# Windere/EAS-SNN

Hardware: AMD Instinct MI355X
Metric: event-frames/sec (T=3) SYOLOX-S Gen1 304x240 (higher is better)
Workload: dtype f32

## Files before the change

eas_snn_amd/csrc/bn_act.hip:

```cpp
#include "eas_common.h"

namespace {

constexpr int NW = EAS_BLOCK / EAS_WAVE;

__device__ __forceinline__ float silu(float z) { return z * eas_sigmoidf(z); }
__device__ __forceinline__ float silu_grad(float z) {
    const float sg = eas_sigmoidf(z);
    return sg * (1.0f + z * (1.0f - sg));
}

__device__ __forceinline__ void bn_silu_fwd_body(const float* __restrict__ y, const float* __restrict__ mean,
                                                 const float* __restrict__ invstd, const float* __restrict__ gamma,
                                                 const float* __restrict__ beta, float* __restrict__ out, int N, int C, int HW, const BnFin& fin,
                                                 int out_ctot, int y_ctot, const int c, const int chunk, const int nchunks_g) {
    __shared__ float st[2];
    if (c >= C) return;
    const int hw4 = HW / EAS_VEC;
    const int64_t groups = (int64_t)N * hw4;
    float mu, istd;
    if (fin.part) {
        bn_finalize_in_block(fin, c, st, mu, istd, chunk == 0);
    } else {
        mu = mean[c];
        istd = invstd[c];
    }
    const float scale = gamma[c] * istd;
    const float shift = beta[c] - mu * scale;
    GroupWalk gw((int64_t)chunk * blockDim.x + threadIdx.x, (int64_t)nchunks_g * blockDim.x, hw4);
    for (int64_t g = (int64_t)chunk * blockDim.x + threadIdx.x; g < groups; g += (int64_t)nchunks_g * blockDim.x, gw.next()) {
        const int64_t n = gw.n;
        const int q = gw.q;
        const int64_t base = (n * C + c) * (int64_t)HW + (int64_t)q * EAS_VEC;
        const float4 v = *reinterpret_cast<const float4*>(y + (y_ctot ? (n * y_ctot + c) * (int64_t)HW + (int64_t)q * EAS_VEC : base));
        float4 o;
        o.x = silu(fmaf(v.x, scale, shift)); o.y = silu(fmaf(v.y, scale, shift));
        o.z = silu(fmaf(v.z, scale, shift)); o.w = silu(fmaf(v.w, scale, shift));
        *reinterpret_cast<float4*>(out + (out_ctot ? (n * out_ctot + c) * (int64_t)HW + (int64_t)q * EAS_VEC : base)) = o;
    }
}

__global__ __launch_bounds__(EAS_BLOCK) void bn_silu_fwd_kernel(const float* __restrict__ y, const float* __restrict__ mean,
                                                                const float* __restrict__ invstd,
                                                                const float* __restrict__ gamma,
                                                                const float* __restrict__ beta, float* __restrict__ out, int N,
                                                                int C, int HW, BnFin fin, int out_ctot, int y_ctot) {
    bn_silu_fwd_body(y, mean, invstd, gamma, beta, out, N, C, HW, fin, out_ctot, y_ctot, (int)(blockIdx.z * 8 + blockIdx.x), (int)blockIdx.y,
                     (int)gridDim.y);
}

template <bool APPLY>
__device__ __forceinline__ void bn_silu_bwd_body(const float* __restrict__ grad_out, const float* __restrict__ y,
                                                 const float* __restrict__ mean, const float* __restrict__ invstd,
                                                 const float* __restrict__ gamma, const float* __restrict__ beta,
                                                 int batch_stats, double* __restrict__ part, int nchunks,
                                                 float* __restrict__ grad_y, float* __restrict__ grad_gamma,
                                                 float* __restrict__ grad_beta, int N, int C, int HW, int go_ctot, int y_ctot, const int c,
                                                 const int chunk, const int nchunks_g) {
    __shared__ double red[NW];
    __shared__ float bc[2];
    if (c >= C) return;
    const float mu = mean[c], istd = invstd[c];
    const float scale = gamma[c] * istd;
    const float shift = beta[c] - mu * scale;
    const int hw4 = HW / EAS_VEC;
    const int64_t groups = (int64_t)N * hw4;
    float m1 = 0.f, m2 = 0.f;
    if (APPLY) bn_bwd_means<2>(part, c, nchunks, (double)N * HW, chunk, batch_stats, grad_beta, grad_gamma, bc, m1, m2);
    float s1 = 0.f, s2 = 0.f;
    GroupWalk gw((int64_t)chunk * blockDim.x + threadIdx.x, (int64_t)nchunks_g * blockDim.x, hw4);
    for (int64_t g = (int64_t)chunk * blockDim.x + threadIdx.x; g < groups; g += (int64_t)nchunks_g * blockDim.x, gw.next()) {
        const int64_t n = gw.n;
        const int q = gw.q;
        const int64_t base = (n * C + c) * (int64_t)HW + (int64_t)q * EAS_VEC;
        const int64_t ybase = y_ctot ? (n * y_ctot + c) * (int64_t)HW + (int64_t)q * EAS_VEC : base;
        const float4 yv = *reinterpret_cast<const float4*>(y + ybase);
        const float4 gv = *reinterpret_cast<const float4*>(grad_out + (go_ctot ? (n * go_ctot + c) * (int64_t)HW + (int64_t)q * EAS_VEC : base));
        const float ys[4] = {yv.x, yv.y, yv.z, yv.w};
        const float gs[4] = {gv.x, gv.y, gv.z, gv.w};
        float o[4];
#pragma unroll
        for (int e = 0; e < 4; ++e) {
            const float dz = gs[e] * silu_grad(fmaf(ys[e], scale, shift));
            const float xhat = bn_xhat(ys[e], mu, istd);
            if (APPLY) {
                o[e] = bn_bwd_apply(scale, dz, xhat, m1, m2);
            } else {
                s1 += dz;
                s2 += dz * xhat;
            }
        }
        if (APPLY) *reinterpret_cast<float4*>(grad_y + ybase) = make_float4(o[0], o[1], o[2], o[3]);
    }
    if (!APPLY) {
        const double t1 = eas_block_sum<double, NW>((double)s1, red);
        const double t2 = eas_block_sum<double, NW>((double)s2, red);
        if (threadIdx.x == 0) {
            part[((int64_t)c * EAS_BN_MAX_CHUNKS + chunk) * 2 + 0] = t1;
            part[((int64_t)c * EAS_BN_MAX_CHUNKS + chunk) * 2 + 1] = t2;
        }
    }
}

template <bool APPLY>
__global__ __launch_bounds__(EAS_BLOCK) void bn_silu_bwd_kernel(const float* __restrict__ grad_out, const float* __restrict__ y,
                                                                const float* __restrict__ mean, const float* __restrict__ invstd,
                                                                const float* __restrict__ gamma, const float* __restrict__ beta,
                                                                int batch_stats, double* __restrict__ part, int nchunks,
                                                                float* __restrict__ grad_y, float* __restrict__ grad_gamma,
                                                                float* __restrict__ grad_beta, int N, int C, int HW, int go_ctot, int y_ctot) {
    bn_silu_bwd_body<APPLY>(grad_out, y, mean, invstd, gamma, beta, batch_stats, part, nchunks, grad_y, grad_gamma, grad_beta, N, C, HW, go_ctot,
                            y_ctot, (int)(blockIdx.z * 8 + blockIdx.x), (int)blockIdx.y, (int)gridDim.y);
}

constexpr int kMaxBnGroup = 12;
struct BnSiluFwdGroup {
    const float* y[kMaxBnGroup];
    const float* mean[kMaxBnGroup];
    const float* invstd[kMaxBnGroup];
    const float* gamma[kMaxBnGroup];
    const float* beta[kMaxBnGroup];
    float* out[kMaxBnGroup];
    BnFin fin[kMaxBnGroup];
    int N[kMaxBnGroup], C[kMaxBnGroup], HW[kMaxBnGroup], out_ctot[kMaxBnGroup], y_ctot[kMaxBnGroup], chunks[kMaxBnGroup];
    int first[kMaxBnGroup + 1];
    int n;
};

template <class G>
__device__ __forceinline__ void bn_group_block(const G& a, int& p, int& c, int& chunk) {
    p = 0;
    for (int i = 1; i < a.n; ++i)
        if ((int)blockIdx.x >= a.first[i]) p = i;
    p = __builtin_amdgcn_readfirstlane(p);
    const int lb = (int)blockIdx.x - a.first[p];
    const int r = lb >> 3;
    chunk = r % a.chunks[p];
    c = (r / a.chunks[p]) * 8 + (lb & 7);
}

__global__ __launch_bounds__(EAS_BLOCK) void bn_silu_fwd_group_kernel(const BnSiluFwdGroup a) {
    int p, c, chunk;
    bn_group_block(a, p, c, chunk);
    bn_silu_fwd_body(a.y[p], a.mean[p], a.invstd[p], a.gamma[p], a.beta[p], a.out[p], a.N[p], a.C[p], a.HW[p], a.fin[p], a.out_ctot[p],
                     a.y_ctot[p], c, chunk, a.chunks[p]);
}

struct BnSiluBwdGroup {
    const float* grad_out[kMaxBnGroup];
    const float* y[kMaxBnGroup];
    const float* mean[kMaxBnGroup];
    const float* invstd[kMaxBnGroup];
// ... 92 lines not shown
    if (q.HW % EAS_VEC != 0 || q.C > 65535) return EAS_ERR_UNSUPPORTED;
    if (((uintptr_t)q.y | (uintptr_t)q.grad_out | (uintptr_t)q.grad_y) & 15) return EAS_ERR_INVALID_ARG;
    return EAS_OK;
}

static inline int bn_chan_blocks(int chunks, int C) { return 8 * chunks * ((C + 7) / 8); }

}

extern "C" {

int eas_bn_silu_fwd_ex(const float* y, float* mean, float* invstd, const float* gamma, const float* beta,
                       float* out, int N, int C, int HW, const EasBnPending* pend, int out_ctot, int y_ctot, eas_stream_t stream) {
    EasBnSiluFwdProblem q{y, mean, invstd, gamma, beta, out, N, C, HW, out_ctot, y_ctot, pend ? *pend : EasBnPending{}};
    BnFin fin;
    if (int rc = bn_silu_fwd_check(q, fin)) return rc;
    EAS_CLEAR_ERR();
    const int chunks = bn_pick_chunks((int64_t)N * (HW / EAS_VEC), C);
    EAS_LAUNCH(bn_silu_fwd_kernel, EAS_CHAN_GRID(chunks, C), dim3(EAS_BLOCK), 0, eas_s(stream), y, mean, invstd, gamma, beta, out, N, C, HW, fin,
               q.out_ctot, q.y_ctot);
    EAS_CHECK_LAUNCH();
    return EAS_OK;
}

int eas_bn_silu_fwd(const float* y, const float* mean, const float* invstd, const float* gamma, const float* beta,
                    float* out, int N, int C, int HW, eas_stream_t stream) {
    return eas_bn_silu_fwd_ex(y, const_cast<float*>(mean), const_cast<float*>(invstd), gamma, beta, out, N, C, HW, nullptr, 0, 0, stream);
}

int eas_bn_silu_bwd(const float* grad_out, const float* y, const float* mean, const float* invstd, const float* gamma,
                    const float* beta, int batch_stats, float* grad_y, float* grad_gamma, float* grad_beta,
                    double* workspace, int N, int C, int HW, int go_ctot, int y_ctot, eas_stream_t stream) {
    EasBnSiluBwdProblem q{grad_out, y, mean, invstd, gamma, beta, grad_y, grad_gamma, grad_beta, workspace, batch_stats, N, C, HW, go_ctot, y_ctot};
    if (int rc = bn_silu_bwd_check(q)) return rc;
    go_ctot = q.grad_out_ctot;
    y_ctot = q.y_ctot;
    hipStream_t st = eas_s(stream);
    EAS_CLEAR_ERR();
    {
        static const bool small_ok = !(eas_dev_env("EAS_BNSILU_BWD") && eas_dev_env("EAS_BNSILU_BWD")[0] == 't');
        constexpr int GPT = 6;
        const int64_t groups = (int64_t)N * (HW / EAS_VEC);
        if (small_ok && C >= 64 && groups <= 1024 * GPT) {
#define EAS_SMALL(NT_) EAS_LAUNCH((bn_silu_bwd_small_kernel<NT_, GPT>), dim3(C), dim3(NT_), 0, st, grad_out, y, mean, invstd, gamma, beta, \
                                           batch_stats, grad_y, grad_gamma, grad_beta, N, C, HW, go_ctot, y_ctot)
            if (groups <= 256 * GPT) EAS_SMALL(256);
            else if (groups <= 512 * GPT) EAS_SMALL(512);
            else EAS_SMALL(1024);
#undef EAS_SMALL
            EAS_CHECK_LAUNCH();
            return EAS_OK;
        }
    }
    const int chunks = bn_pick_chunks((int64_t)N * (HW / EAS_VEC), C);
    EAS_LAUNCH(bn_silu_bwd_kernel<false>, EAS_CHAN_GRID(chunks, C), dim3(EAS_BLOCK), 0, st, grad_out, y, mean, invstd, gamma, beta,
                       batch_stats, workspace, chunks, grad_y, grad_gamma, grad_beta, N, C, HW, go_ctot, y_ctot);
    EAS_CHECK_LAUNCH();
    EAS_LAUNCH(bn_silu_bwd_kernel<true>, EAS_CHAN_GRID(chunks, C), dim3(EAS_BLOCK), 0, st, grad_out, y, mean, invstd, gamma, beta,
                       batch_stats, workspace, chunks, grad_y, grad_gamma, grad_beta, N, C, HW, go_ctot, y_ctot);
    EAS_CHECK_LAUNCH();
    return EAS_OK;
}

int eas_bn_silu_fwd_group(const EasBnSiluFwdProblem* pr, int n, eas_stream_t stream) {
    if (!pr || n < 1) return EAS_ERR_INVALID_ARG;
    if (n > kMaxBnGroup) return EAS_ERR_UNSUPPORTED;
    BnSiluFwdGroup a{};
    int blocks = 0;
    for (int p = 0; p < n; ++p) {
        EasBnSiluFwdProblem q = pr[p];
        if (int rc = bn_silu_fwd_check(q, a.fin[p])) return rc;
        a.y[p] = q.y; a.mean[p] = q.mean; a.invstd[p] = q.invstd; a.gamma[p] = q.gamma; a.beta[p] = q.beta; a.out[p] = q.out;
        a.N[p] = q.N; a.C[p] = q.C; a.HW[p] = q.HW; a.out_ctot[p] = q.out_ctot; a.y_ctot[p] = q.y_ctot;
        a.chunks[p] = bn_pick_chunks((int64_t)q.N * (q.HW / EAS_VEC), q.C);
        a.first[p] = blocks;
        blocks += bn_chan_blocks(a.chunks[p], q.C);
    }
    a.first[n] = blocks;
    a.n = n;
    EAS_CLEAR_ERR();
    EAS_LAUNCH(bn_silu_fwd_group_kernel, dim3(blocks), dim3(EAS_BLOCK), 0, eas_s(stream), a);
    EAS_CHECK_LAUNCH();
    return EAS_OK;
}

int eas_bn_silu_bwd_group(const EasBnSiluBwdProblem* pr, int n, eas_stream_t stream) {
    if (!pr || n < 1) return EAS_ERR_INVALID_ARG;
    if (n > kMaxBnGroup) return EAS_ERR_UNSUPPORTED;
    BnSiluBwdGroup a{};
    int blocks = 0;
    for (int p = 0; p < n; ++p) {
        EasBnSiluBwdProblem q = pr[p];
        if (int rc = bn_silu_bwd_check(q)) return rc;
        a.grad_out[p] = q.grad_out; a.y[p] = q.y; a.mean[p] = q.mean; a.invstd[p] = q.invstd; a.gamma[p] = q.gamma; a.beta[p] = q.beta;
        a.part[p] = q.workspace; a.grad_y[p] = q.grad_y; a.grad_gamma[p] = q.grad_gamma; a.grad_beta[p] = q.grad_beta;
        a.batch_stats[p] = q.batch_stats; a.N[p] = q.N; a.C[p] = q.C; a.HW[p] = q.HW; a.go_ctot[p] = q.grad_out_ctot; a.y_ctot[p] = q.y_ctot;
        a.chunks[p] = bn_pick_chunks((int64_t)q.N * (q.HW / EAS_VEC), q.C);
        a.first[p] = blocks;
        blocks += bn_chan_blocks(a.chunks[p], q.C);
    }
    a.first[n] = blocks;
    a.n = n;
    EAS_CLEAR_ERR();
    EAS_LAUNCH(bn_silu_bwd_group_kernel<false>, dim3(blocks), dim3(EAS_BLOCK), 0, eas_s(stream), a);
    EAS_CHECK_LAUNCH();
    EAS_LAUNCH(bn_silu_bwd_group_kernel<true>, dim3(blocks), dim3(EAS_BLOCK), 0, eas_s(stream), a);
    EAS_CHECK_LAUNCH();
    return EAS_OK;
}

}
```

eas_snn_amd/csrc/bn_lif.hip:

```cpp
#include <stdlib.h>
#include <string.h>

#include "bn_lif_policy.h"
#include "eas_common.h"

namespace {

constexpr int NW = EAS_BLOCK / EAS_WAVE;

__global__ __launch_bounds__(EAS_BLOCK) void bn_stats_partial(const float* __restrict__ y, int TN, int C, int HW,
                                                              double* __restrict__ part, int Cy) {
    __shared__ double red[NW];
    const int c = blockIdx.y;
    const int hw4 = HW / EAS_VEC;
    const int64_t groups = (int64_t)TN * hw4;
    double s = 0.0, ss = 0.0;
    const int64_t stride = (int64_t)gridDim.x * blockDim.x;
    GroupWalk gw((int64_t)blockIdx.x * blockDim.x + threadIdx.x, stride, hw4);
    int64_t g = (int64_t)blockIdx.x * blockDim.x + threadIdx.x;
    for (; g + stride < groups; g += 2 * stride) {
        const float4 v0 = reinterpret_cast<const float4*>(y + (((int64_t)gw.n * Cy + c) * (int64_t)HW))[gw.q];
        gw.next();
        const float4 v1 = reinterpret_cast<const float4*>(y + (((int64_t)gw.n * Cy + c) * (int64_t)HW))[gw.q];
        gw.next();
// ... 185 lines not shown
                    acc[j][e] += s;
                    if (res_planes) s += (float)rp[e][j];
                    o[j] = (__bf16)s;
                }
                planes[(((int64_t)t * N + n) * out_groups_tot + grp) * (int64_t)HW + (int64_t)q * PV + e] = o;
            }
        }
#pragma unroll
        for (int j = 0; j < 8; ++j) {
            const int64_t base = (n * C + 8 * grp + j) * (int64_t)HW + (int64_t)q * PV;
            if (v_out) {
                vecp o;
#pragma unroll
                for (int e = 0; e < PV; ++e) o[e] = v[j][e];
                *reinterpret_cast<vecp*>(v_out + base) = o;
            }
            if (mean_out) {
                vecp o;
#pragma unroll
                for (int e = 0; e < PV; ++e) o[e] = acc[j][e] / Tf;
                *reinterpret_cast<vecp*>(mean_out + base) = o;
            }
        }
    }
}

template <int T_, bool HARD, bool DI, bool STRICT, class POL>
__device__ __forceinline__ void recompute_dz(const float (&yv)[T_], const float (&gs)[T_], float v0, float scale,
                                             float shift, float k, float omk, const EasLifParams& p, bool detach,
                                             int sg_id, float alpha, float (&dz)[T_], float& dk, float& da) {
    float h[T_], vprev[T_], z[T_];
    float v = v0;
#pragma unroll
    for (int t = 0; t < T_; ++t) {
        float s;
        vprev[t] = v;
        z[t] = fmaf(yv[t], scale, shift);
        eas_lif_step<HARD, DI, STRICT>(v, z[t], k, omk, p.v_th, p.v_reset, h[t], s);
    }
    float gv = 0.f;
#pragma unroll
    for (int t = T_ - 1; t >= 0; --t) {
        float dkt, gx;
        if constexpr (POL::fast)
            eas_lif_step_bwd_ct<HARD, DI, STRICT, POL::sg, POL::detach>(gs[t], gv, h[t], vprev[t], z[t], k, omk, p.v_th, p.v_reset, alpha, dkt,
                                                                        gx, da);
        else
            eas_lif_step_bwd<HARD, DI, STRICT>(gs[t], gv, h[t], vprev[t], z[t], k, omk, p.v_th, p.v_reset, detach, sg_id, alpha, dkt, gx, da);
        dz[t] = gx;
        dk += dkt;
    }
}

template <int T_, bool HARD, bool DI, bool STRICT, bool APPLY, class POL>
__global__ __launch_bounds__(EAS_BLOCK) void bn_lif_bwd_kernel(
    const float* __restrict__ grad_s, const float* __restrict__ grad_mean, const float* __restrict__ y,
    const float* __restrict__ mean, const float* __restrict__ invstd, const float* __restrict__ gamma,
    const float* __restrict__ beta, const float* __restrict__ v_init, EasLifParams p, int sg_id, float alpha,
    int batch_stats, double* __restrict__ part, int nchunks, float* __restrict__ grad_y, float* __restrict__ grad_gamma,
    float* __restrict__ grad_beta, float* __restrict__ grad_w, int N, int C, int HW, int bcast, int gs_ctot, int y_ctot,
    const float* __restrict__ alpha_dev, float* __restrict__ grad_alpha, int c_begin, int c_end, int finalize) {
    __shared__ double red[NW];
    __shared__ float bc[2];
    constexpr bool FAST = POL::fast;
    if (FAST) { bcast = 0; sg_id = POL::sg; }
    if (alpha_dev) alpha = fabsf(*alpha_dev);
    const int c = c_begin + blockIdx.z * 8 + blockIdx.x;
    if (c >= c_end) return;
    const int chunk = blockIdx.y, nchunks_g = gridDim.y;
    const float mu = mean[c], istd = invstd[c];
    const float scale = gamma[c] * istd;
    const float shift = beta[c] - mu * scale;
    const float k = eas_lif_k(p);
    const float omk = 1.0f - k;
    const bool detach = (p.flags & EAS_LIF_DETACH_RESET) != 0;
    const int hw4 = HW / EAS_VEC;
    const int64_t groups = (int64_t)N * hw4;
    const int64_t M = (int64_t)N * C * HW;
    const float invT = 1.0f / (float)T_;
    const int Cy = y_ctot ? y_ctot : C;
    const int64_t My = (int64_t)N * Cy * HW;
    const int64_t yts = bcast ? 0 : My;
    const int64_t Mg = gs_ctot ? (int64_t)N * gs_ctot * HW : M;
    const int Cg = gs_ctot ? gs_ctot : C;
    float m1 = 0.f, m2 = 0.f;
    if (APPLY) bn_bwd_means<4>(part, c, nchunks, (double)T_ * N * HW, chunk, batch_stats, grad_beta, grad_gamma, bc, m1, m2);
    float s1 = 0.f, s2 = 0.f, dk = 0.f, da = 0.f;
    GroupWalk gw((int64_t)chunk * blockDim.x + threadIdx.x, (int64_t)nchunks_g * blockDim.x, hw4);
    for (int64_t g = (int64_t)chunk * blockDim.x + threadIdx.x; g < groups; g += (int64_t)nchunks_g * blockDim.x, gw.next()) {
        const int64_t n = gw.n;
        const int q = gw.q;
        const int64_t base = (n * C + c) * (int64_t)HW + (int64_t)q * EAS_VEC;
        float4 ys[T_], gsv[T_];
        const int64_t ybase = (n * Cy + c) * (int64_t)HW + (int64_t)q * EAS_VEC;
#pragma unroll
        for (int t = 0; t < T_; ++t) ys[t] = *reinterpret_cast<const float4*>(y + (int64_t)t * yts + ybase);
        float4 gm = make_float4(0.f, 0.f, 0.f, 0.f);
        if (!FAST && grad_mean) {
            gm = *reinterpret_cast<const float4*>(grad_mean + base);
            gm.x *= invT; gm.y *= invT; gm.z *= invT; gm.w *= invT;
        }
#pragma unroll
        for (int t = 0; t < T_; ++t) {
            gsv[t] = gm;
            if (FAST || grad_s) {
                const int64_t gbase = FAST ? (n * Cg + c) * (int64_t)HW + (int64_t)q * EAS_VEC
                                           : (gs_ctot ? (n * gs_ctot + c) * (int64_t)HW + (int64_t)q * EAS_VEC : base);
                const float4 g4 = *reinterpret_cast<const float4*>(grad_s + (int64_t)t * Mg + gbase);
                gsv[t].x += g4.x; gsv[t].y += g4.y; gsv[t].z += g4.z; gsv[t].w += g4.w;
            }
        }
        const float vr0 = HARD ? p.v_reset : 0.0f;
        float4 v0 = make_float4(vr0, vr0, vr0, vr0);
        if (!FAST && v_init) v0 = *reinterpret_cast<const float4*>(v_init + base);
        float4 outv[T_];
#pragma unroll
        for (int e = 0; e < EAS_VEC; ++e) {
            float yv[T_], gs[T_], dz[T_];
#pragma unroll
            for (int t = 0; t < T_; ++t) {
                yv[t] = reinterpret_cast<const float*>(&ys[t])[e];
                gs[t] = reinterpret_cast<const float*>(&gsv[t])[e];
            }
            const float v0e = reinterpret_cast<const float*>(&v0)[e];
            float dke = 0.f;
            recompute_dz<T_, HARD, DI, STRICT, POL>(yv, gs, v0e, scale, shift, k, omk, p, detach, sg_id, alpha, dz, dke, da);
#pragma unroll
            for (int t = 0; t < T_; ++t) {
                const float xhat = bn_xhat(yv[t], mu, istd);
                if (APPLY) {
                    reinterpret_cast<float*>(&outv[t])[e] = bn_bwd_apply(scale, dz[t], xhat, m1, m2);
                } else {
                    s1 += dz[t];
                    s2 += dz[t] * xhat;
                }
            }
            dk += dke;
        }
        if (APPLY) {
            if (bcast) {
                float4 a = outv[0];
#pragma unroll
                for (int t = 1; t < T_; ++t) { a.x += outv[t].x; a.y += outv[t].y; a.z += outv[t].z; a.w += outv[t].w; }
                *reinterpret_cast<float4*>(grad_y + ybase) = a;
            } else {
#pragma unroll
                for (int t = 0; t < T_; ++t) *reinterpret_cast<float4*>(grad_y + (int64_t)t * My + ybase) = outv[t];
            }
        }
    }
    if (APPLY && finalize && chunk == 0 && c == c_begin) {
        auto slot = [&](int i, int k_) {
            const int cc = i / nchunks, j = i - cc * nchunks;
            return part[((int64_t)cc * EAS_BN_MAX_CHUNKS + j) * 4 + k_];
        };
        eas_lif_scalar_grads(C * nchunks, [&](int i) { return slot(i, 2); }, [&](int i) { return slot(i, 3); }, p.w_logit, alpha_dev, grad_w,
                             grad_alpha, red);
    }
    if (!APPLY) {
        const double t1 = eas_block_sum<double, NW>((double)s1, red);
        const double t2 = eas_block_sum<double, NW>((double)s2, red);
        const double t3 = eas_block_sum<double, NW>((double)dk, red);
        double t4 = 0.0;
        if (sg_id == EAS_SG_PATAN) t4 = eas_block_sum<double, NW>((double)da, red);
        if (threadIdx.x == 0) {
            double* o = part + ((int64_t)c * EAS_BN_MAX_CHUNKS + chunk) * 4;
            o[0] = t1; o[1] = t2; o[2] = t3; o[3] = t4;
        }
    }
}

template <int T_, bool HARD, bool DI, bool STRICT, int NT_, int GPT, class POL>
__global__ __launch_bounds__(NT_) void bn_lif_bwd_small_kernel(
    const float* __restrict__ grad_s, const float* __restrict__ grad_mean, const float* __restrict__ y,
    const float* __restrict__ mean, const float* __restrict__ invstd, const float* __restrict__ gamma,
    const float* __restrict__ beta, const float* __restrict__ v_init, EasLifParams p, int sg_id, float alpha,
    int batch_stats, double* __restrict__ part, float* __restrict__ grad_y, float* __restrict__ grad_gamma,
    float* __restrict__ grad_beta, int N, int C, int HW, int gs_ctot, int y_ctot, const float* __restrict__ alpha_dev) {
    constexpr int NWV = NT_ / EAS_WAVE;
    __shared__ double red[4][NWV];
    __shared__ float bc[2];
    if (POL::fast) sg_id = POL::sg;
    if (alpha_dev) alpha = fabsf(*alpha_dev);
    const int c = blockIdx.x;
    const float mu = mean[c], istd = invstd[c];
    const float scale = gamma[c] * istd;
    const float shift = beta[c] - mu * scale;
    const float k = eas_lif_k(p);
    const float omk = 1.0f - k;
    const bool detach = (p.flags & EAS_LIF_DETACH_RESET) != 0;
    const int hw4 = HW / EAS_VEC;
    const int groups = N * hw4;
    const int64_t M = (int64_t)N * C * HW;
    const int Cy = y_ctot ? y_ctot : C;
    const int64_t My = (int64_t)N * Cy * HW;
    const int64_t Mg = gs_ctot ? (int64_t)N * gs_ctot * HW : M;
    const float invT = 1.0f / (float)T_;
    float4 ys[GPT][T_], gsv[GPT][T_], v0[GPT];
    int64_t ybase[GPT];
#pragma unroll
    for (int i = 0; i < GPT; ++i) {
        const int g = threadIdx.x + i * NT_;
        const int gg = g < groups ? g : groups - 1;
        const int n = gg / hw4, q = gg - n * hw4;
        const int64_t base = ((int64_t)n * C + c) * (int64_t)HW + (int64_t)q * EAS_VEC;
        ybase[i] = ((int64_t)n * Cy + c) * (int64_t)HW + (int64_t)q * EAS_VEC;
#pragma unroll
        for (int t = 0; t < T_; ++t) ys[i][t] = *reinterpret_cast<const float4*>(y + (int64_t)t * My + ybase[i]);
        float4 gm = make_float4(0.f, 0.f, 0.f, 0.f);
        if (grad_mean) {
            gm = *reinterpret_cast<const float4*>(grad_mean + base);
            gm.x *= invT; gm.y *= invT; gm.z *= invT; gm.w *= invT;
        }
#pragma unroll
        for (int t = 0; t < T_; ++t) {
            gsv[i][t] = gm;
            if (grad_s) {
                const int64_t gbase = gs_ctot ? ((int64_t)n * gs_ctot + c) * (int64_t)HW + (int64_t)q * EAS_VEC : base;
                const float4 g4 = *reinterpret_cast<const float4*>(grad_s + (int64_t)t * Mg + gbase);
                gsv[i][t].x += g4.x; gsv[i][t].y += g4.y; gsv[i][t].z += g4.z; gsv[i][t].w += g4.w;
            }
        }
        const float vr0 = HARD ? p.v_reset : 0.0f;
        v0[i] = make_float4(vr0, vr0, vr0, vr0);
        if (v_init) v0[i] = *reinterpret_cast<const float4*>(v_init + base);
    }
    float sum[4] = {0.f, 0.f, 0.f, 0.f};
#pragma unroll
    for (int i = 0; i < GPT; ++i) {
        const bool live = threadIdx.x + i * NT_ < groups;
#pragma unroll
        for (int e = 0; e < EAS_VEC; ++e) {
            float yv[T_], gs[T_], dz[T_];
#pragma unroll
            for (int t = 0; t < T_; ++t) {
                yv[t] = reinterpret_cast<const float*>(&ys[i][t])[e];
                gs[t] = reinterpret_cast<const float*>(&gsv[i][t])[e];
            }
            float dke = 0.f, dae = 0.f;
            recompute_dz<T_, HARD, DI, STRICT, POL>(yv, gs, reinterpret_cast<const float*>(&v0[i])[e], scale, shift, k, omk, p, detach, sg_id, alpha, dz, dke, dae);
            if (live) {
#pragma unroll
                for (int t = 0; t < T_; ++t) {
                    sum[0] += dz[t];
                    sum[1] += dz[t] * bn_xhat(yv[t], mu, istd);
                }
                sum[2] += dke;
                sum[3] += dae;
            }
        }
    }
    double t[4];
    eas_block_totals<NWV, 4>(sum, red, t);
    if (threadIdx.x == 0) {
        bn_bwd_publish(t[0], t[1], (double)T_ * N * HW, true, c, grad_beta, grad_gamma, bc);
        double* o = part + ((int64_t)c * EAS_BN_MAX_CHUNKS) * 4;
        o[0] = t[0]; o[1] = t[1]; o[2] = t[2]; o[3] = sg_id == EAS_SG_PATAN ? t[3] : 0.0;
    }
    __syncthreads();
    const float m1 = batch_stats ? bc[0] : 0.f, m2 = batch_stats ? bc[1] : 0.f;
#pragma unroll
    for (int i = 0; i < GPT; ++i) {
        if (threadIdx.x + i * NT_ >= groups) continue;
        float4 outv[T_];
#pragma unroll
        for (int e = 0; e < EAS_VEC; ++e) {
            float yv[T_], gs[T_], dz[T_];
#pragma unroll
            for (int t = 0; t < T_; ++t) {
                yv[t] = reinterpret_cast<const float*>(&ys[i][t])[e];
                gs[t] = reinterpret_cast<const float*>(&gsv[i][t])[e];
            }
            float dke = 0.f, dae = 0.f;
            recompute_dz<T_, HARD, DI, STRICT, POL>(yv, gs, reinterpret_cast<const float*>(&v0[i])[e], scale, shift, k, omk, p, detach, sg_id, alpha, dz, dke, dae);
#pragma unroll
            for (int t = 0; t < T_; ++t) reinterpret_cast<float*>(&outv[t])[e] = bn_bwd_apply(scale, dz[t], bn_xhat(yv[t], mu, istd), m1, m2);
        }
#pragma unroll
        for (int t = 0; t < T_; ++t) *reinterpret_cast<float4*>(grad_y + (int64_t)t * My + ybase[i]) = outv[t];
    }
}

__global__ __launch_bounds__(EAS_BLOCK) void bn_lif_bwd_scalars_kernel(const double* __restrict__ part, int C, EasLifParams p, float* __restrict__ grad_w,
                                                                       const float* __restrict__ alpha_dev, float* __restrict__ grad_alpha) {
    __shared__ double red[NW];
    auto slot = [&](int i, int k_) { return part[((int64_t)i * EAS_BN_MAX_CHUNKS) * 4 + k_]; };
    eas_lif_scalar_grads(C, [&](int i) { return slot(i, 2); }, [&](int i) { return slot(i, 3); }, p.w_logit, alpha_dev, grad_w, grad_alpha, red);
}

template <int T_, bool HARD, bool DI, bool STRICT>
int launch_fwd_t(const float* y, const float* mean, const float* invstd, const float* gamma, const float* beta,
                 const float* v_in, float* v_out, EasLifParams p, float* spikes, float* mean_out, int N, int C, int HW,
                 int bcast, const BnFin& fin, const BnLifOut& ox, bf16x8* planes, const bf16x8* res_planes, int out_groups, int res_groups,
                 hipStream_t st) {
    if (planes) {
        if (fin.part) {
            EAS_LAUNCH(bn_finalize_kernel, dim3(C), dim3(EAS_BLOCK), 0, st, fin);
            EAS_CHECK_LAUNCH();
        }
        constexpr int PV = 1;
        const int chunks = bn_pick_chunks((int64_t)N * (HW / PV), C / 8);
        EAS_LAUNCH((bn_lif_fwd_sp_kernel<T_, HARD, DI, STRICT, PV>), EAS_CHAN_GRID(chunks, C / 8), dim3(EAS_BLOCK), 0, st, y,
                           mean, invstd, gamma, beta, v_in,
                           v_out, p, planes, res_planes, mean_out, N, C, HW, bcast, ox.y_ctot, out_groups, res_groups);
        EAS_CHECK_LAUNCH();
        return EAS_OK;
    }
    const int chunks = bn_pick_chunks((int64_t)N * (HW / EAS_VEC), C);
    EAS_LAUNCH((bn_lif_fwd_kernel<T_, HARD, DI, STRICT>), EAS_CHAN_GRID(chunks, C), dim3(EAS_BLOCK), 0, st, y, mean,
                       invstd, gamma, beta, v_in, v_out, p, spikes, mean_out, N, C, HW, bcast, fin, ox);
    EAS_CHECK_LAUNCH();
    return EAS_OK;
}

template <bool HARD, bool DI, bool STRICT>
int launch_fwd(int T, const float* y, const float* mean, const float* invstd, const float* gamma, const float* beta,
               const float* v_in, float* v_out, EasLifParams p, float* spikes, float* mean_out, int N, int C, int HW,
               int bcast, const BnFin& fin, const BnLifOut& ox, bf16x8* planes, const bf16x8* res_planes, int out_groups, int res_groups,
               hipStream_t st) {
#define EAS_CASE(TT) \
    case TT: return launch_fwd_t<TT, HARD, DI, STRICT>(y, mean, invstd, gamma, beta, v_in, v_out, p, spikes, mean_out, N, C, HW, bcast, fin, ox, planes, res_planes, out_groups, res_groups, st);
    switch (T) {
        EAS_CASE(1) EAS_CASE(2) EAS_CASE(3) EAS_CASE(4) EAS_CASE(5) EAS_CASE(6) EAS_CASE(7) EAS_CASE(8)
        default: return EAS_ERR_UNSUPPORTED;
    }
#undef EAS_CASE
}

struct BwdCall {
    const float *grad_s, *grad_mean, *y, *mean, *invstd, *gamma, *beta, *v_init;
    EasLifParams p;
    int sg;
    float alpha;
    int batch_stats;
    float *grad_y, *grad_gamma, *grad_beta, *grad_w;
    double* ws;
    int T, N, C, HW, bcast, gs_ctot, y_ctot;
    const float* alpha_dev;
    float* grad_alpha;
    hipStream_t st;
};

static inline bool bwd_form(const char* word) {
    const char* form = getenv("EAS_BNLIF_BWD");
    return form && strstr(form, word);
}

static inline int bwd_one_pass_gpt(const BwdCall& c) {
    const int gpt = c.T <= 3 ? 3 : (c.T <= 5 ? 2 : 1);
    const int64_t groups = (int64_t)c.N * (c.HW / EAS_VEC);
    return (!bwd_form("two") && !c.bcast && c.C >= 64 && groups <= 512 * gpt) ? gpt : 0;
}

template <int T_, bool HARD, bool DI, bool STRICT, class POL>
int launch_bwd_t(const BwdCall& c) {
    const int N = c.N, C = c.C, HW = c.HW;
    const int chunks = bn_pick_chunks((int64_t)N * (HW / EAS_VEC), C);
    if (bwd_one_pass_gpt(c)) {
        constexpr int GPT = T_ <= 3 ? 3 : (T_ <= 5 ? 2 : 1);
        const int64_t groups = (int64_t)N * (HW / EAS_VEC);
#define EAS_SMALL(NT_) EAS_LAUNCH((bn_lif_bwd_small_kernel<T_, HARD, DI, STRICT, NT_, GPT, POL>), dim3(C), dim3(NT_), 0, c.st, c.grad_s, c.grad_mean, c.y, \
                                   c.mean, c.invstd, c.gamma, c.beta, c.v_init, c.p, c.sg, c.alpha, c.batch_stats, c.ws, c.grad_y, c.grad_gamma,       \
                                   c.grad_beta, N, C, HW, c.gs_ctot, c.y_ctot, c.alpha_dev)
        if (groups <= 256 * GPT) EAS_SMALL(256);
        else EAS_SMALL(512);
#undef EAS_SMALL
        EAS_CHECK_LAUNCH();
        if (c.grad_w || c.grad_alpha) {
            EAS_LAUNCH(bn_lif_bwd_scalars_kernel, dim3(1), dim3(EAS_BLOCK), 0, c.st, c.ws, C, c.p, c.grad_w, c.alpha_dev, c.grad_alpha);
            EAS_CHECK_LAUNCH();
        }
        return EAS_OK;
    }
    static const int group_mb = eas_dev_env("EAS_BNLIF_BWD_GROUP_MB") ? atoi(eas_dev_env("EAS_BNLIF_BWD_GROUP_MB")) : 0;
    int gc = C;
    if (group_mb > 0) {
        const double per_channel = (double)N * HW * 4.0 * ((c.bcast ? 1 : T_) + T_);
        gc = (int)(group_mb * 1048576.0 / per_channel) / 8 * 8;
        if (gc < 8) gc = 8;
        if (gc > C) gc = C;
    }
    for (int c0 = 0; c0 < C; c0 += gc) {
        const int c1 = c0 + gc < C ? c0 + gc : C;
        const int last = c1 == C;
        EAS_LAUNCH((bn_lif_bwd_kernel<T_, HARD, DI, STRICT, false, POL>), EAS_CHAN_GRID(chunks, c1 - c0), dim3(EAS_BLOCK), 0, c.st, c.grad_s,
                   c.grad_mean, c.y, c.mean, c.invstd, c.gamma, c.beta, c.v_init, c.p, c.sg, c.alpha, c.batch_stats, c.ws, chunks, c.grad_y,
                   c.grad_gamma, c.grad_beta, (float*)nullptr, N, C, HW, c.bcast, c.gs_ctot, c.y_ctot, c.alpha_dev, (float*)nullptr, c0, c1, 0);
        EAS_CHECK_LAUNCH();
        EAS_LAUNCH((bn_lif_bwd_kernel<T_, HARD, DI, STRICT, true, POL>), EAS_CHAN_GRID(chunks, c1 - c0), dim3(EAS_BLOCK), 0, c.st, c.grad_s,
                   c.grad_mean, c.y, c.mean, c.invstd, c.gamma, c.beta, c.v_init, c.p, c.sg, c.alpha, c.batch_stats, c.ws, chunks, c.grad_y,
                   c.grad_gamma, c.grad_beta, c.grad_w, N, C, HW, c.bcast, c.gs_ctot, c.y_ctot, c.alpha_dev, c.grad_alpha, c0, c1, last);
        EAS_CHECK_LAUNCH();
    }
    return EAS_OK;
}

struct BwdRow {
    int T;
    bool hard, di;
    int sg;
    bool detach;
    int (*fn)(const BwdCall&);
};
template <int T_, bool HARD, bool DI, int SG = EAS_SG_RUNTIME, bool DETACH = false>
constexpr BwdRow bwd_row() {
    return {T_, HARD, DI, SG, DETACH, launch_bwd_t<T_, HARD, DI, false, BnLifBwdPolicy<SG, DETACH>>};
}
#define EAS_BWD_GENERIC_ROWS(H, D) \
    bwd_row<1, H, D>(), bwd_row<2, H, D>(), bwd_row<3, H, D>(), bwd_row<4, H, D>(), bwd_row<5, H, D>(), bwd_row<6, H, D>(), bwd_row<7, H, D>(), bwd_row<8, H, D>()
const BwdRow kBwdInstances[] = {
    bwd_row<3, false, false, EAS_SG_ATAN>(), bwd_row<5, false, false, EAS_SG_ATAN>(), bwd_row<7, false, false, EAS_SG_ATAN>(),
    EAS_BWD_GENERIC_ROWS(false, false), EAS_BWD_GENERIC_ROWS(true, false), EAS_BWD_GENERIC_ROWS(false, true), EAS_BWD_GENERIC_ROWS(true, true),
};
#undef EAS_BWD_GENERIC_ROWS

int bwd_select(const BwdCall& c) {
    const bool hard = c.p.flags & EAS_LIF_HARD_RESET, di = c.p.flags & EAS_LIF_DECAY_INPUT, detach = c.p.flags & EAS_LIF_DETACH_RESET;
    if (c.p.flags & EAS_LIF_FIRE_STRICT) return EAS_ERR_UNSUPPORTED;
    const bool plain = bwd_one_pass_gpt(c) || (c.grad_s && !c.grad_mean && !c.v_init && !c.bcast);
    const bool fast_ok = plain && !bwd_form("generic");
    for (const BwdRow& r : kBwdInstances) {
        if (r.T != c.T || r.hard != hard || r.di != di) continue;
        if (r.sg == EAS_SG_RUNTIME || (fast_ok && r.sg == c.sg && r.detach == detach)) return r.fn(c);
    }
    return EAS_ERR_UNSUPPORTED;
}
// ... 143 lines not shown
```

eas_snn_amd/csrc/eas_common.h:

```cpp
#pragma once
#include <hip/hip_runtime.h>
#include <stdint.h>
#include <stdlib.h>

#include <type_traits>

#include "../../include/eas_hip.h"

#define EAS_WAVE 64
#define EAS_BLOCK 256

#define EAS_CLEAR_ERR() (void)hipGetLastError()
#define EAS_CHECK_LAUNCH()                                          \
    do {                                                            \
        if (hipGetLastError() != hipSuccess) return EAS_ERR_LAUNCH; \
    } while (0)

static inline hipStream_t eas_s(eas_stream_t s) { return reinterpret_cast<hipStream_t>(s); }

__attribute__((visibility("hidden"))) extern int eas_trace_on;
__attribute__((visibility("hidden"))) extern long long eas_launch_count;
__attribute__((visibility("hidden"))) void eas_trace_kernel(const void* host_function);
#define EAS_LAUNCH(kern, ...)                                                \
    do {                                                                     \
// ... 118 lines not shown
                    s[p] += a;
                    q[p] = __builtin_elementwise_fma(a, a, q[p]);
                }
        }
#pragma unroll
        for (int stat = 0; stat < 2; ++stat) {
#pragma unroll
            for (int e = 0; e < 16; ++e) {
                const f2 v = stat ? q[e >> 1] : s[e >> 1];
                scratch[(4 * h + (e & 3) + 8 * (e >> 2)) * EAS_STATS_PITCH + r] = (e & 1) ? v.y : v.x;
            }
            __builtin_amdgcn_fence(__ATOMIC_RELEASE, "wavefront");
            __builtin_amdgcn_wave_barrier();
            __builtin_amdgcn_fence(__ATOMIC_ACQUIRE, "wavefront");
            if (lane < 32) {
                const float4* row = reinterpret_cast<const float4*>(scratch + lane * EAS_STATS_PITCH);
                double t = 0.0;
#pragma unroll
                for (int k = 0; k < 8; ++k) {
                    const float4 v = row[k];
                    t += (double)v.x; t += (double)v.y; t += (double)v.z; t += (double)v.w;
                }
                red[(m * 32 + lane) * 2 + stat] = t;
            }
            __builtin_amdgcn_fence(__ATOMIC_RELEASE, "wavefront");
            __builtin_amdgcn_wave_barrier();
            __builtin_amdgcn_fence(__ATOMIC_ACQUIRE, "wavefront");
        }
    }
}

__device__ __forceinline__ void eas_conv_stats_store(const double* red, int wave_stride, int nwv, int t, int co, int Cout, double* stats, int nb,
                                                     int block) {
    if (co >= Cout) return;
    double s = 0.0, q = 0.0;
    for (int w = 0; w < nwv; ++w) {
        s += red[w * wave_stride + t * 2 + 0];
        q += red[w * wave_stride + t * 2 + 1];
    }
    *reinterpret_cast<double2*>(stats + ((int64_t)co * nb + block) * 2) = make_double2(s, q);
}

#define EAS_VEC 4
#define EAS_BN_MAX_CHUNKS 64

static inline int bn_pick_chunks(int64_t groups_per_channel, int C) {
    int64_t want = (groups_per_channel + EAS_BLOCK - 1) / EAS_BLOCK;
    int64_t cap = 8192 / (C > 0 ? C : 1);
    if (cap < 1) cap = 1;
    if (cap > EAS_BN_MAX_CHUNKS) cap = EAS_BN_MAX_CHUNKS;
    if (want > cap) want = cap;
    if (want < 1) want = 1;
    return (int)want;
}

static inline bool bn_slice(int& ctot, int C) {
    if (ctot == C) ctot = 0;
    return ctot == 0 || ctot > C;
}

struct BnFin {
    const double* part;
    int nchunks, pitch, replicas;
    double count;
    float eps, momentum;
    float* mean_out;
    float* invstd_out;
    float* rmean;
    float* rvar;
};

static inline int bn_fin_from(const EasBnPending* pend, float* mean, float* invstd, BnFin& fin) {
    fin = BnFin{};
    if (!pend || !pend->partial) return EAS_OK;
    const int pitch = pend->pitch ? pend->pitch : EAS_BN_MAX_CHUNKS;
    if (pend->chunks < 1 || pend->chunks > pitch || pend->pitch < 0 || !(pend->count >= 1.0) || pend->replicas < 1) return EAS_ERR_INVALID_ARG;
    if ((pend->running_mean == nullptr) != (pend->running_var == nullptr)) return EAS_ERR_INVALID_ARG;
    fin = BnFin{pend->partial, pend->chunks, pitch, pend->replicas, pend->count, pend->eps, pend->momentum, mean, invstd, pend->running_mean,
                pend->running_var};
    return EAS_OK;
}

template <int SLOTS>
__device__ __forceinline__ void bn_wave_partials(const double* __restrict__ part, int64_t first, int n, double& a, double& b) {
    a = 0.0;
    b = 0.0;
    if ((int)threadIdx.x < n) {
        a = part[(first + threadIdx.x) * SLOTS + 0];
        b = part[(first + threadIdx.x) * SLOTS + 1];
    }
    a = eas_wave_sum(a);
    b = eas_wave_sum(b);
}

__device__ __forceinline__ void bn_from_totals(const BnFin& f, int c, double s, double ss, bool publish, float& mu, float& istd) {
    const double m = s / f.count;
    double var = ss / f.count - m * m;
    if (var < 0.0) var = 0.0;
    mu = (float)m;
    istd = (float)(1.0 / sqrt(var + (double)f.eps));
    if (publish) {
        f.mean_out[c] = mu;
        f.invstd_out[c] = istd;
        if (f.rmean) {
            const double full = f.count * f.replicas;
            const double unbiased = full > 1.0 ? var * full / (full - 1.0) : var;
// ... 187 lines not shown
```

Before: 3406.

## Prefetch next group in BN backward loops and size chunks by occupancy

BN-SiLU and BN-LIF backward kernels now software-pipeline their grid-stride loops: the next group's loads are issued before the current group is computed, and the first load is hoisted above the mean-broadcast prologue. Chunk count per channel is now chosen from the device CU count and the kernels' measured occupancy instead of a fixed 8192/C cap. Block reductions are fused into one multi-value reduction, and the one-pass LIF kernel stores dz so the apply phase no longer recomputes it. The prefetch raises register pressure, and the new chunk count changes the grid size and the reduction order.

```diff
diff --git a/eas_snn_amd/csrc/bn_act.hip b/eas_snn_amd/csrc/bn_act.hip
--- a/eas_snn_amd/csrc/bn_act.hip
+++ b/eas_snn_amd/csrc/bn_act.hip
@@ -57,7 +57,7 @@
                                                  float* __restrict__ grad_y, float* __restrict__ grad_gamma,
                                                  float* __restrict__ grad_beta, int N, int C, int HW, int go_ctot, int y_ctot, const int c,
                                                  const int chunk, const int nchunks_g) {
-    __shared__ double red[NW];
+    __shared__ double red[2][NW];
     __shared__ float bc[2];
     if (c >= C) return;
     const float mu = mean[c], istd = invstd[c];
@@ -65,17 +65,28 @@
     const float shift = beta[c] - mu * scale;
     const int hw4 = HW / EAS_VEC;
     const int64_t groups = (int64_t)N * hw4;
+    struct Group {
+        float4 yv, gv;
+        int64_t ybase;
+    };
+    auto load = [&](const GroupWalk& w, Group& r) {
+        const int64_t n = w.n;
+        const int q = w.q;
+        const int64_t base = (n * C + c) * (int64_t)HW + (int64_t)q * EAS_VEC;
+        r.ybase = y_ctot ? (n * y_ctot + c) * (int64_t)HW + (int64_t)q * EAS_VEC : base;
+        r.yv = *reinterpret_cast<const float4*>(y + r.ybase);
+        r.gv = *reinterpret_cast<const float4*>(grad_out + (go_ctot ? (n * go_ctot + c) * (int64_t)HW + (int64_t)q * EAS_VEC : base));
+    };
+    const int64_t stride = (int64_t)nchunks_g * blockDim.x;
+    int64_t g = (int64_t)chunk * blockDim.x + threadIdx.x;
+    GroupWalk gw(g, stride, hw4);
+    Group cur{}, nxt{};
+    if (g < groups) load(gw, cur);
     float m1 = 0.f, m2 = 0.f;
     if (APPLY) bn_bwd_means<2>(part, c, nchunks, (double)N * HW, chunk, batch_stats, grad_beta, grad_gamma, bc, m1, m2);
     float s1 = 0.f, s2 = 0.f;
-    GroupWalk gw((int64_t)chunk * blockDim.x + threadIdx.x, (int64_t)nchunks_g * blockDim.x, hw4);
-    for (int64_t g = (int64_t)chunk * blockDim.x + threadIdx.x; g < groups; g += (int64_t)nchunks_g * blockDim.x, gw.next()) {
-        const int64_t n = gw.n;
-        const int q = gw.q;
-        const int64_t base = (n * C + c) * (int64_t)HW + (int64_t)q * EAS_VEC;
-        const int64_t ybase = y_ctot ? (n * y_ctot + c) * (int64_t)HW + (int64_t)q * EAS_VEC : base;
-        const float4 yv = *reinterpret_cast<const float4*>(y + ybase);
-        const float4 gv = *reinterpret_cast<const float4*>(grad_out + (go_ctot ? (n * go_ctot + c) * (int64_t)HW + (int64_t)q * EAS_VEC : base));
+    auto consume = [&](const Group& r) {
+        const float4 yv = r.yv, gv = r.gv;
         const float ys[4] = {yv.x, yv.y, yv.z, yv.w};
         const float gs[4] = {gv.x, gv.y, gv.z, gv.w};
         float o[4];
@@ -90,14 +101,22 @@
                 s2 += dz * xhat;
             }
         }
-        if (APPLY) *reinterpret_cast<float4*>(grad_y + ybase) = make_float4(o[0], o[1], o[2], o[3]);
-    }
+        if (APPLY) *reinterpret_cast<float4*>(grad_y + r.ybase) = make_float4(o[0], o[1], o[2], o[3]);
+    };
+    for (; g + stride < groups; g += stride) {
+        gw.next();
+        load(gw, nxt);
+        consume(cur);
+        cur = nxt;
+    }
+    if (g < groups) consume(cur);
     if (!APPLY) {
-        const double t1 = eas_block_sum<double, NW>((double)s1, red);
-        const double t2 = eas_block_sum<double, NW>((double)s2, red);
+        const float sum[2] = {s1, s2};
+        double t[2];
+        eas_block_totals<NW, 2>(sum, red, t);
         if (threadIdx.x == 0) {
-            part[((int64_t)c * EAS_BN_MAX_CHUNKS + chunk) * 2 + 0] = t1;
-            part[((int64_t)c * EAS_BN_MAX_CHUNKS + chunk) * 2 + 1] = t2;
+            part[((int64_t)c * EAS_BN_MAX_CHUNKS + chunk) * 2 + 0] = t[0];
+            part[((int64_t)c * EAS_BN_MAX_CHUNKS + chunk) * 2 + 1] = t[1];
         }
     }
 }
@@ -296,7 +315,8 @@
             return EAS_OK;
         }
     }
-    const int chunks = bn_pick_chunks((int64_t)N * (HW / EAS_VEC), C);
+    const BnChip chip = bn_chip<bn_silu_bwd_kernel<false>, bn_silu_bwd_kernel<true>>();
+    const int chunks = bn_pick_chunks_bwd((int64_t)N * (HW / EAS_VEC), C, chip.resident, chip.cus);
     EAS_LAUNCH(bn_silu_bwd_kernel<false>, EAS_CHAN_GRID(chunks, C), dim3(EAS_BLOCK), 0, st, grad_out, y, mean, invstd, gamma, beta,
                        batch_stats, workspace, chunks, grad_y, grad_gamma, grad_beta, N, C, HW, go_ctot, y_ctot);
     EAS_CHECK_LAUNCH();
@@ -333,13 +353,18 @@
     if (n > kMaxBnGroup) return EAS_ERR_UNSUPPORTED;
     BnSiluBwdGroup a{};
     int blocks = 0;
+    const BnChip chip = bn_chip<bn_silu_bwd_group_kernel<false>, bn_silu_bwd_group_kernel<true>>();
+    double total = 0.0;
+    for (int p = 0; p < n; ++p)
+        if (pr[p].N > 0 && pr[p].C > 0 && pr[p].HW > 0) total += (double)pr[p].N * pr[p].C * pr[p].HW;
     for (int p = 0; p < n; ++p) {
         EasBnSiluBwdProblem q = pr[p];
         if (int rc = bn_silu_bwd_check(q)) return rc;
+        const double share = (double)q.N * q.C * q.HW / total;
         a.grad_out[p] = q.grad_out; a.y[p] = q.y; a.mean[p] = q.mean; a.invstd[p] = q.invstd; a.gamma[p] = q.gamma; a.beta[p] = q.beta;
         a.part[p] = q.workspace; a.grad_y[p] = q.grad_y; a.grad_gamma[p] = q.grad_gamma; a.grad_beta[p] = q.grad_beta;
         a.batch_stats[p] = q.batch_stats; a.N[p] = q.N; a.C[p] = q.C; a.HW[p] = q.HW; a.go_ctot[p] = q.grad_out_ctot; a.y_ctot[p] = q.y_ctot;
-        a.chunks[p] = bn_pick_chunks((int64_t)q.N * (q.HW / EAS_VEC), q.C);
+        a.chunks[p] = bn_pick_chunks_bwd((int64_t)q.N * (q.HW / EAS_VEC), q.C, (int64_t)(chip.resident * share), (int64_t)(chip.cus * share) + 1);
         a.first[p] = blocks;
         blocks += bn_chan_blocks(a.chunks[p], q.C);
     }
diff --git a/eas_snn_amd/csrc/bn_lif.hip b/eas_snn_amd/csrc/bn_lif.hip
--- a/eas_snn_amd/csrc/bn_lif.hip
+++ b/eas_snn_amd/csrc/bn_lif.hip
@@ -261,6 +261,16 @@
     }
 }
 
+template <int T_>
+struct BwdGroup {
+    float4 ys[T_], gs[T_], gm, v0;
+    int64_t ybase;
+};
+#ifndef EAS_BN_BWD_TWO_SETS_MAX_T
+#define EAS_BN_BWD_TWO_SETS_MAX_T 3
+#endif
+constexpr bool bwd_two_sets(int T) { return T <= EAS_BN_BWD_TWO_SETS_MAX_T; }
+
 template <int T_, bool HARD, bool DI, bool STRICT, bool APPLY, class POL>
 __global__ __launch_bounds__(EAS_BLOCK) void bn_lif_bwd_kernel(
     const float* __restrict__ grad_s, const float* __restrict__ grad_mean, const float* __restrict__ y,
@@ -269,7 +279,7 @@
     int batch_stats, double* __restrict__ part, int nchunks, float* __restrict__ grad_y, float* __restrict__ grad_gamma,
     float* __restrict__ grad_beta, float* __restrict__ grad_w, int N, int C, int HW, int bcast, int gs_ctot, int y_ctot,
     const float* __restrict__ alpha_dev, float* __restrict__ grad_alpha, int c_begin, int c_end, int finalize) {
-    __shared__ double red[NW];
+    __shared__ double red[4][NW];
     __shared__ float bc[2];
     constexpr bool FAST = POL::fast;
     if (FAST) { bcast = 0; sg_id = POL::sg; }
@@ -292,36 +302,50 @@
     const int64_t yts = bcast ? 0 : My;
     const int64_t Mg = gs_ctot ? (int64_t)N * gs_ctot * HW : M;
     const int Cg = gs_ctot ? gs_ctot : C;
+    auto load = [&](const GroupWalk& w, BwdGroup<T_>& r) {
+        const int64_t n = w.n;
+        const int q = w.q;
+        const int64_t base = (n * C + c) * (int64_t)HW + (int64_t)q * EAS_VEC;
+        r.ybase = (n * Cy + c) * (int64_t)HW + (int64_t)q * EAS_VEC;
+#pragma unroll
+        for (int t = 0; t < T_; ++t) r.ys[t] = *reinterpret_cast<const float4*>(y + (int64_t)t * yts + r.ybase);
+        if (!FAST && grad_mean) r.gm = *reinterpret_cast<const float4*>(grad_mean + base);
+        if (FAST || grad_s) {
+            const int64_t gbase = FAST ? (n * Cg + c) * (int64_t)HW + (int64_t)q * EAS_VEC
+                                       : (gs_ctot ? (n * gs_ctot + c) * (int64_t)HW + (int64_t)q * EAS_VEC : base);
+#pragma unroll
+            for (int t = 0; t < T_; ++t) r.gs[t] = *reinterpret_cast<const float4*>(grad_s + (int64_t)t * Mg + gbase);
+        }
+        if (!FAST && v_init) r.v0 = *reinterpret_cast<const float4*>(v_init + base);
+    };
+    const int64_t stride = (int64_t)nchunks_g * blockDim.x;
+    int64_t g = (int64_t)chunk * blockDim.x + threadIdx.x;
+    GroupWalk gw(g, stride, hw4);
+    BwdGroup<T_> cur{}, nxt{};
+    if (g < groups) load(gw, cur);
     float m1 = 0.f, m2 = 0.f;
     if (APPLY) bn_bwd_means<4>(part, c, nchunks, (double)T_ * N * HW, chunk, batch_stats, grad_beta, grad_gamma, bc, m1, m2);
     float s1 = 0.f, s2 = 0.f, dk = 0.f, da = 0.f;
-    GroupWalk gw((int64_t)chunk * blockDim.x + threadIdx.x, (int64_t)nchunks_g * blockDim.x, hw4);
-    for (int64_t g = (int64_t)chunk * blockDim.x + threadIdx.x; g < groups; g += (int64_t)nchunks_g * blockDim.x, gw.next()) {
-        const int64_t n = gw.n;
-        const int q = gw.q;
-        const int64_t base = (n * C + c) * (int64_t)HW + (int64_t)q * EAS_VEC;
-        float4 ys[T_], gsv[T_];
-        const int64_t ybase = (n * Cy + c) * (int64_t)HW + (int64_t)q * EAS_VEC;
-#pragma unroll
-        for (int t = 0; t < T_; ++t) ys[t] = *reinterpret_cast<const float4*>(y + (int64_t)t * yts + ybase);
+    auto consume = [&](const BwdGroup<T_>& r) {
+        const float4(&ys)[T_] = r.ys;
+        const int64_t ybase = r.ybase;
+        float4 gsv[T_];
         float4 gm = make_float4(0.f, 0.f, 0.f, 0.f);
         if (!FAST && grad_mean) {
-            gm = *reinterpret_cast<const float4*>(grad_mean + base);
+            gm = r.gm;
             gm.x *= invT; gm.y *= invT; gm.z *= invT; gm.w *= invT;
         }
 #pragma unroll
         for (int t = 0; t < T_; ++t) {
             gsv[t] = gm;
             if (FAST || grad_s) {
-                const int64_t gbase = FAST ? (n * Cg + c) * (int64_t)HW + (int64_t)q * EAS_VEC
-                                           : (gs_ctot ? (n * gs_ctot + c) * (int64_t)HW + (int64_t)q * EAS_VEC : base);
-                const float4 g4 = *reinterpret_cast<const float4*>(grad_s + (int64_t)t * Mg + gbase);
+                const float4 g4 = r.gs[t];
                 gsv[t].x += g4.x; gsv[t].y += g4.y; gsv[t].z += g4.z; gsv[t].w += g4.w;
             }
         }
         const float vr0 = HARD ? p.v_reset : 0.0f;
         float4 v0 = make_float4(vr0, vr0, vr0, vr0);
-        if (!FAST && v_init) v0 = *reinterpret_cast<const float4*>(v_init + base);
+        if (!FAST && v_init) v0 = r.v0;
         float4 outv[T_];
 #pragma unroll
         for (int e = 0; e < EAS_VEC; ++e) {
@@ -357,6 +381,21 @@
                 for (int t = 0; t < T_; ++t) *reinterpret_cast<float4*>(grad_y + (int64_t)t * My + ybase) = outv[t];
             }
         }
+    };
+    if (bwd_two_sets(T_)) {
+        for (; g + stride < groups; g += stride) {
+            gw.next();
+            load(gw, nxt);
+            consume(cur);
+            cur = nxt;
+        }
+        if (g < groups) consume(cur);
+    } else {
+        for (; g < groups; g += stride) {
+            consume(cur);
+            gw.next();
+            if (g + stride < groups) load(gw, cur);
+        }
     }
     if (APPLY && finalize && chunk == 0 && c == c_begin) {
         auto slot = [&](int i, int k_) {
@@ -364,17 +403,15 @@
             return part[((int64_t)cc * EAS_BN_MAX_CHUNKS + j) * 4 + k_];
         };
         eas_lif_scalar_grads(C * nchunks, [&](int i) { return slot(i, 2); }, [&](int i) { return slot(i, 3); }, p.w_logit, alpha_dev, grad_w,
-                             grad_alpha, red);
+                             grad_alpha, red[0]);
     }
     if (!APPLY) {
-        const double t1 = eas_block_sum<double, NW>((double)s1, red);
-        const double t2 = eas_block_sum<double, NW>((double)s2, red);
-        const double t3 = eas_block_sum<double, NW>((double)dk, red);
-        double t4 = 0.0;
-        if (sg_id == EAS_SG_PATAN) t4 = eas_block_sum<double, NW>((double)da, red);
+        const float sum[4] = {s1, s2, dk, da};
+        double t[4];
+        eas_block_totals<NW, 4>(sum, red, t);
         if (threadIdx.x == 0) {
             double* o = part + ((int64_t)c * EAS_BN_MAX_CHUNKS + chunk) * 4;
-            o[0] = t1; o[1] = t2; o[2] = t3; o[3] = t4;
+            o[0] = t[0]; o[1] = t[1]; o[2] = t[2]; o[3] = sg_id == EAS_SG_PATAN ? t[3] : 0.0;
         }
     }
 }
@@ -457,6 +494,8 @@
                 sum[2] += dke;
                 sum[3] += dae;
             }
+#pragma unroll
+            for (int t = 0; t < T_; ++t) reinterpret_cast<float*>(&gsv[i][t])[e] = dz[t];
         }
     }
     double t[4];
@@ -474,16 +513,10 @@
         float4 outv[T_];
 #pragma unroll
         for (int e = 0; e < EAS_VEC; ++e) {
-            float yv[T_], gs[T_], dz[T_];
-#pragma unroll
-            for (int t = 0; t < T_; ++t) {
-                yv[t] = reinterpret_cast<const float*>(&ys[i][t])[e];
-                gs[t] = reinterpret_cast<const float*>(&gsv[i][t])[e];
-            }
-            float dke = 0.f, dae = 0.f;
-            recompute_dz<T_, HARD, DI, STRICT, POL>(yv, gs, reinterpret_cast<const float*>(&v0[i])[e], scale, shift, k, omk, p, detach, sg_id, alpha, dz, dke, dae);
-#pragma unroll
-            for (int t = 0; t < T_; ++t) reinterpret_cast<float*>(&outv[t])[e] = bn_bwd_apply(scale, dz[t], bn_xhat(yv[t], mu, istd), m1, m2);
+#pragma unroll
+            for (int t = 0; t < T_; ++t)
+                reinterpret_cast<float*>(&outv[t])[e] = bn_bwd_apply(scale, reinterpret_cast<const float*>(&gsv[i][t])[e],
+                                                                     bn_xhat(reinterpret_cast<const float*>(&ys[i][t])[e], mu, istd), m1, m2);
         }
 #pragma unroll
         for (int t = 0; t < T_; ++t) *reinterpret_cast<float4*>(grad_y + (int64_t)t * My + ybase[i]) = outv[t];
@@ -564,7 +597,6 @@
 template <int T_, bool HARD, bool DI, bool STRICT, class POL>
 int launch_bwd_t(const BwdCall& c) {
     const int N = c.N, C = c.C, HW = c.HW;
-    const int chunks = bn_pick_chunks((int64_t)N * (HW / EAS_VEC), C);
     if (bwd_one_pass_gpt(c)) {
         constexpr int GPT = T_ <= 3 ? 3 : (T_ <= 5 ? 2 : 1);
         const int64_t groups = (int64_t)N * (HW / EAS_VEC);
@@ -581,6 +613,8 @@
         }
         return EAS_OK;
     }
+    const BnChip chip = bn_chip<bn_lif_bwd_kernel<T_, HARD, DI, STRICT, false, POL>, bn_lif_bwd_kernel<T_, HARD, DI, STRICT, true, POL>>();
+    const int chunks = bn_pick_chunks_bwd((int64_t)N * (HW / EAS_VEC), C, chip.resident, chip.cus);
     static const int group_mb = eas_dev_env("EAS_BNLIF_BWD_GROUP_MB") ? atoi(eas_dev_env("EAS_BNLIF_BWD_GROUP_MB")) : 0;
     int gc = C;
     if (group_mb > 0) {
diff --git a/eas_snn_amd/csrc/eas_common.h b/eas_snn_amd/csrc/eas_common.h
--- a/eas_snn_amd/csrc/eas_common.h
+++ b/eas_snn_amd/csrc/eas_common.h
@@ -194,6 +194,45 @@
     if (want > cap) want = cap;
     if (want < 1) want = 1;
     return (int)want;
+}
+
+#ifndef EAS_BN_BWD_ROUNDS
+#define EAS_BN_BWD_ROUNDS 1
+#endif
+#define EAS_BN_BWD_MAX_WALK 20
+static inline int bn_pick_chunks_bwd(int64_t groups_per_channel, int C, int64_t resident, int64_t cus) {
+    if (const char* force = getenv("EAS_BN_BWD_CHUNKS")) {
+        const int v = atoi(force);
+        if (v >= 1) return v < EAS_BN_MAX_CHUNKS ? v : EAS_BN_MAX_CHUNKS;
+    }
+    if (C < 1) C = 1;
+    const int64_t one = (groups_per_channel + EAS_BLOCK - 1) / EAS_BLOCK;
+    const int64_t busy = (cus + C - 1) / C, walk = (one + EAS_BN_BWD_MAX_WALK - 1) / EAS_BN_BWD_MAX_WALK;
+    int64_t chunks = EAS_BN_BWD_ROUNDS * resident / C;
+    if (chunks < busy) chunks = busy;
+    if (chunks < walk) chunks = walk;
+    if (chunks > one) chunks = one;
+    if (chunks > EAS_BN_MAX_CHUNKS) chunks = EAS_BN_MAX_CHUNKS;
+    if (chunks < 1) chunks = 1;
+    return (int)chunks;
+}
+
+struct BnChip {
+    int64_t cus, resident;
+};
+template <auto... KERNS>
+static inline BnChip bn_chip() {
+    static BnChip chip{0, 0};
+    if (chip.cus > 0) return chip;
+    int dev = 0, cus = 0, per_cu = 1 << 30;
+    if (hipGetDevice(&dev) != hipSuccess || hipDeviceGetAttribute(&cus, hipDeviceAttributeMultiprocessorCount, dev) != hipSuccess || cus < 1) cus = 1;
+    for (const void* k : {(const void*)KERNS...}) {
+        int n = 0;
+        if (hipOccupancyMaxActiveBlocksPerMultiprocessor(&n, k, EAS_BLOCK, 0) != hipSuccess || n < 1) n = 1;
+        if (n < per_cu) per_cu = n;
+    }
+    chip = BnChip{cus, (int64_t)cus * per_cu};
+    return chip;
 }
 
 static inline bool bn_slice(int& ctot, int C) {
```

Measured after the change: 3415 (median of 6 runs). No clear change (+0.3%).
